# HpWang-whu/YOHO

Measured on AMD Instinct MI355X. Metric: keypoints/sec (5000 kp x60 rot desc+YOHO-O), higher is better.
Workload: dtype fp16x2 split (2^-22-accurate products, fp32 accumulate); 1 GPU

## Files before the change

### yoho_amd/csrc/api.hip

```cpp
#include "common.h"
#include <cstdarg>
#include <cstdio>
#include <cstring>
#include <cstdlib>
#include <cmath>
#include <vector>

namespace yoho {

static thread_local char g_err[512] = "";

void set_error(const char* fmt, ...) {
    va_list ap;
    va_start(ap, fmt);
    vsnprintf(g_err, sizeof(g_err), fmt, ap);
    va_end(ap);
}

void clear_error() { g_err[0] = 0; }

int hip_fail(hipError_t e, const char* what, const char* file, int line) {
    set_error("HIP error %d (%s) at %s:%d: %s", (int)e, hipGetErrorString(e), file, line, what);
    return YOHO_EHIP;
}
// ... 247 lines not shown
                const int* pr = p32.data() + (a < G ? a : G - 1) * G + 4 * q;
                pq[q * 64 + a] = (unsigned)pr[0] | ((unsigned)pr[1] << 8) | ((unsigned)pr[2] << 16) | ((unsigned)pr[3] << 24);
            }
        if ((rc = upload(pq.data(), sizeof(unsigned) * pq.size(), (void**)&c->dPq))) { delete c; return rc; }
    }
    {
        int e = -1;
        for (int g = 0; g < G && e < 0; ++g) {
            float d = 0.f;
            for (int i = 0; i < 9; ++i) d += std::fabs(R[g * 9 + i] - ((i % 4 == 0) ? 1.f : 0.f));
            if (d < 1e-4f) e = g;
        }
        bool ok = e >= 0;
        for (int k = 0; k < NTAP && ok; ++k) {
            const int nk = N[e * NTAP + k];
            int k2 = -1;
            for (int j = 0; j < NTAP; ++j) if (N[nk * NTAP + j] == e) k2 = j;
            if (k2 < 0) ok = false; else c->tap_inv[k] = k2;
        }
        if (!ok) for (int k = 0; k < NTAP; ++k) c->tap_inv[k] = -1;
        if ((rc = upload(c->tap_inv, sizeof(int) * NTAP, (void**)&c->d_tap_inv))) { delete c; return rc; }
    }
    std::vector<int> slab(NCFG * NTAP * G, 0), outg(NCFG * G, -1);
    auto fill = [&](int cfg, const std::vector<int>& glist, int gpw, bool replicate) {
        const int nslots = 4 * gpw;
        for (int sl = 0; sl < nslots; ++sl) {
            int g = -1;
            if (replicate) g = glist[0];
            else if (sl < (int)glist.size()) g = glist[sl];
            outg[cfg * G + sl] = g;
        }
        for (int tap = 0; tap < NTAP; ++tap)
            for (int sl = 0; sl < nslots; ++sl) {
                const int g = outg[cfg * G + sl];
                slab[cfg * NTAP * G + tap * nslots + sl] = (g < 0 ? 0 : (int)N[g * NTAP + tap]) * 1024;
            }
    };
    std::vector<int> all(G); for (int i = 0; i < G; ++i) all[i] = i;
    std::vector<int> one(NTAP); for (int k = 0; k < NTAP; ++k) one[k] = N[k];
    std::vector<bool> in2(G, false);
    for (int k = 0; k < NTAP; ++k) for (int k2 = 0; k2 < NTAP; ++k2) in2[N[one[k] * NTAP + k2]] = true;
    std::vector<int> two; for (int g = 0; g < G; ++g) if (in2[g]) two.push_back(g);
    if (two.size() > 48) { set_error("2-hop cone of group element 0 has %zu > 48 elements", two.size()); delete c; return YOHO_EINVAL; }
    fill(CFG_FULL, all, 15, false);
    fill(CFG_C45, two, 12, false);
    fill(CFG_C13, one, 4, false);
    fill(CFG_C1, std::vector<int>{0}, 1, true);
    if ((rc = upload_slot_tables(slab.data(), outg.data(), c->tabs)) || (rc = gconv_init())) { delete c; return rc; }
    {
        std::vector<int> slab4(3 * 7 * 32, 0), unitg(3 * 32 * 2, -1);
        const std::vector<int>* lists[3] = {&all, &two, &one};
        for (int cfg = 0; cfg < 3; ++cfg) {
            const std::vector<int>& gl = *lists[cfg];
            int* ug = &unitg[cfg * 64];
            for (size_t k = 0; k < gl.size(); ++k) ug[k] = gl[k];
            for (int tp = 0; tp < 7; ++tp)
                for (int u = 0; u < 32; ++u)
                    for (int gs = 0; gs < 2; ++gs)
                        for (int h = 0; h < 2; ++h) {
                            int g = ug[2 * u + gs];
                            if (g < 0) g = ug[2 * u];
                            int tap = 2 * tp + h;
                            if (tap >= NTAP) tap = 2 * tp;
                            slab4[(cfg * 7 + tp) * 32 + u] |= (g < 0 ? 0 : (int)N[g * NTAP + tap]) << (8 * (2 * gs + h));
                        }
        }
        if ((rc = upload_slot_tables16(slab4.data(), unitg.data(), c->tabs)) || (rc = gconv16_init())) { delete c; return rc; }
    }
    c->gconv_mode = 4;
    c->partII_mode = 2;
    {
        auto is = [](const char* name, const char* val) { const char* e = std::getenv(name); return e && std::strcmp(e, val) == 0; };
        auto num = [](const char* name) { const char* e = std::getenv(name); return e ? std::atoi(e) : 0; };
        c->env.partII_tail_staged = is("YOHO_PARTII_TAIL", "staged");
        c->env.transfer_staged = is("YOHO_TRANSFER", "staged");
        c->env.xf_steal = !is("YOHO_XF_STEAL", "0");
        c->env.nn_splits = num("YOHO_NN_SPLITS");
        c->env.fcgf_f32 = is("YOHO_FCGF", "f32");
        c->env.fcgf_full_maps = is("YOHO_FCGF_MAPS", "full");
        c->env.fcgf_norm_staged = is("YOHO_FCGF_NORM", "staged");
        c->env.fcgf_heads_staged = is("YOHO_FCGF_HEADS", "staged");
        if (const char* e = std::getenv("YOHO_WS_LIMIT_MB")) c->env.ws_limit_mb = std::atoll(e);
        if (is("YOHO_PARTII_L1", "3")) c->env.partII_l1_variant = FG_TILE256_W8;
    }
    if (const char* m = std::getenv("YOHO_FCGF_CELLS")) c->fcgf_cell_sort = std::atoi(m);
    if (const char* m = std::getenv("YOHO_FCGF_SORT")) c->fcgf_parity_sort = std::strcmp(m, "0") == 0 ? 0 : 1;
    if (const char* m = std::getenv("YOHO_FCGF_COORDS")) c->fcgf_hash_coords = std::strcmp(m, "hash") == 0 ? 1 : 0;
    if (const char* m = std::getenv("YOHO_NN")) c->nn_prefilter = std::strcmp(m, "brute") == 0 ? 0 : 1;
    if (const char* m = std::getenv("YOHO_PARTII")) c->partII_mode = std::strcmp(m, "f32") == 0 ? 0 : (std::strcmp(m, "fp16x2") == 0 ? 2 : (std::strcmp(m, "cgemm") == 0 ? 3 : (std::strcmp(m, "cgemm8") == 0 ? 4 : 1)));
    if (const char* m = std::getenv("YOHO_PARTI_CHUNK")) {
        int ck = 0, ns = 1;
        if (std::sscanf(m, "%dx%d", &ck, &ns) >= 1 && ck >= 0 && (ns == 1 || ns == 2)) { c->partI_chunk = (ck + 255) / 256 * 256; c->partI_streams = ns; }
    }
    if (const char* m = std::getenv("YOHO_GCONV")) c->gconv_mode = std::strcmp(m, "f32") == 0 ? 0 : (std::strcmp(m, "bf16x3") == 0 ? 1 : (std::strcmp(m, "fp16x2") == 0 ? 3 : (std::strcmp(m, "fgemm") == 0 ? 4 : (std::strcmp(m, "fgemm256") == 0 ? 5 : (std::strcmp(m, "fgemm128") == 0 ? 6 : (std::strcmp(m, "fgemm8") == 0 ? 7 : 2))))));
    c->fb = new FourierBasis();
    if ((rc = build_fourier(N, P, *c->fb))) { delete c->fb; delete c; return rc; }
    {
        std::vector<float> fpad(2 * 64 * 64, 0.f);
        for (int s = 0; s < G; ++s)
            for (int g = 0; g < G; ++g) {
                fpad[s * 64 + g] = (float)c->fb->F[s * G + g];
                fpad[64 * 64 + g * 64 + s] = (float)c->fb->F[s * G + g];
            }
        if ((rc = upload(fpad.data(), fpad.size() * sizeof(float), (void**)&c->dFpad)) || (rc = gft_init()) || (rc = fgemm_init()) || (rc = gft16_init())) { delete c->fb; delete c; return rc; }
        std::vector<unsigned short> f16;
        build_gft16_frags(*c->fb, f16);
        if ((rc = upload(f16.data(), f16.size() * sizeof(unsigned short), &c->dF16))) { delete c->fb; delete c; return rc; }
        hipDeviceProp_t prop;
        if (hipGetDeviceProperties(&prop, device) == hipSuccess && prop.multiProcessorCount > 0) c->nCU = prop.multiProcessorCount;
    }
    HIPCHK(hipMalloc((void**)&c->d_rflag, 4 * sizeof(int)));
    HIPCHK(hipMemset(c->d_rflag, 0, 4 * sizeof(int)));
    HIPCHK(hipMalloc((void**)&c->d_amax, 12 * sizeof(unsigned)));
    HIPCHK(hipMemset(c->d_amax, 0, 12 * sizeof(unsigned)));
    {
        for (int g = 0; g < G; ++g) c->cone_slot_of[g] = -1;
        for (int j = 0; j < NTAP; ++j)
            for (int k = 0; k < NTAP; ++k) c->cone_slot_of[c->hN[c->hN[j] * NTAP + k]] = 0;
        int ns = 0;
        for (int g = 0; g < G; ++g) if (c->cone_slot_of[g] == 0) c->cone_slot_of[g] = ns++;
        c->cone_nslot = ns;
        for (int j = 0; j < NTAP; ++j) {
            c->cone_outg[j] = c->hN[j];
            for (int k = 0; k < NTAP; ++k) c->cone_slot[j * 13 + k] = (unsigned char)c->cone_slot_of[c->hN[c->hN[j] * NTAP + k]];
        }
    }
    HIPCHK(hipMalloc((void**)&c->d_xfctr, 16 * sizeof(int)));
    HIPCHK(hipMemset(c->d_xfctr, 0, 16 * sizeof(int)));
    *out = c;
    return 0;
}

int yoho_ctx_destroy(yoho_ctx* c) {
    if (!c) return 0;
    (void)hipSetDevice(c->device);
    (void)hipDeviceSynchronize();
    for (auto& L : c->p1) free_layer(L);
    for (auto& L : c->p2) free_layer(L);
    if (c->p2_init_bn_s) (void)hipFree(c->p2_init_bn_s);
    if (c->p2_init_bn_t) (void)hipFree(c->p2_init_bn_t);
    if (c->ws.p) (void)hipFree(c->ws.p);
    if (c->dR32) (void)hipFree(c->dR32);
    if (c->dR64) (void)hipFree(c->dR64);
    if (c->dN) (void)hipFree(c->dN);
    if (c->dP) (void)hipFree(c->dP);
    if (c->dPq) (void)hipFree(c->dPq);
    if (c->pair_ws) (void)hipFree(c->pair_ws);
    if (c->pair_host) (void)hipHostFree(c->pair_host);
    if (c->dFpad) (void)hipFree(c->dFpad);
    if (c->dF16) (void)hipFree(c->dF16);
    if (c->fcgf) fcgf_free(c->fcgf);
    if (c->d_tap_inv) (void)hipFree(c->d_tap_inv);
    if (c->d_rflag) (void)hipFree(c->d_rflag);
    if (c->d_xfctr) (void)hipFree(c->d_xfctr);
    if (c->d_amax) (void)hipFree(c->d_amax);
    for (int* t : {c->tabs.slabtab, c->tabs.outg, c->tabs.slab4, c->tabs.unitg}) if (t) (void)hipFree(t);
    delete c->fb;
    for (auto& e : c->ev) (void)hipEventDestroy(e);
    for (auto& e : c->ev_pass) if (e) (void)hipEventDestroy(e);
    for (auto& e : c->phase.pool) (void)hipEventDestroy(e);
    if (c->ev_fork) (void)hipEventDestroy(c->ev_fork);
    if (c->ev_join) (void)hipEventDestroy(c->ev_join);
    if (c->side_stream) (void)hipStreamDestroy(c->side_stream);
    delete c;
    return 0;
}

int yoho_load_partI(yoho_ctx* c, const yoho_partI_weights* w) {
    if (!c || !w) { set_error("yoho_load_partI: null argument"); return YOHO_EINVAL; }
    HIPCHK(hipSetDevice(c->device));
    c->has_partI = false;
    int rc;
    if ((rc = build_layer(c->p1[0], w->conv_in, 32, 256, NTAP, &w->res_in_bn, c->fb))) return rc;
    if ((rc = build_layer(c->p1[1], w->res_in, 256, 512, NTAP, &w->res_out_bn, c->fb))) return rc;
    if ((rc = build_layer(c->p1[2], w->res_out, 512, 256, NTAP, &w->out_bn, c->fb))) return rc;
    if ((rc = build_layer(c->p1[3], w->conv_out, 256, 32, NTAP, nullptr, c->fb))) return rc;
    for (auto& L : c->p1) L.tabs = &c->tabs;
    c->has_partI = true;
    return 0;
}

int yoho_load_partII(yoho_ctx* c, const yoho_partII_weights* w) {
    if (!c || !w) { set_error("yoho_load_partII: null argument"); return YOHO_EINVAL; }
    HIPCHK(hipSetDevice(c->device));
    c->has_partII = false;
    int rc;
    std::vector<float> s, t;
    if (!w->init_bn.gamma || !w->init_bn.beta || !w->init_bn.mean || !w->init_bn.var) { set_error("null batch-norm pointer"); return YOHO_EINVAL; }
    bn_affine(w->init_bn, 128, 128, s, t);
    if (c->p2_init_bn_s) { (void)hipFree(c->p2_init_bn_s); c->p2_init_bn_s = nullptr; }
    if (c->p2_init_bn_t) { (void)hipFree(c->p2_init_bn_t); c->p2_init_bn_t = nullptr; }
    if ((rc = upload(s.data(), 128 * sizeof(float), (void**)&c->p2_init_bn_s))) return rc;
    if ((rc = upload(t.data(), 128 * sizeof(float), (void**)&c->p2_init_bn_t))) return rc;
    if ((rc = build_layer(c->p2[0], w->init, 128, 256, NTAP, &w->res_in_bn, c->fb))) return rc;
    if ((rc = build_layer(c->p2[1], w->res_in, 256, 512, NTAP, &w->res_out_bn))) return rc;
    {
        std::vector<unsigned short> wc, wc8;
        if (pack_cgemm_weights(w->res_in.weight, 256, 512, NTAP, wc, &c->p2[1].wcg_descale, wc8)) { set_error("cone-GEMM weight packing failed"); return YOHO_EINVAL; }
        if ((rc = upload(wc.data(), wc.size() * sizeof(unsigned short), &c->p2[1].wcg))) return rc;
        if ((rc = upload(wc8.data(), wc8.size() * sizeof(unsigned short), &c->p2[1].wcg8))) return rc;
    }
    if ((rc = build_layer(c->p2[2], w->res_out, 512, 256, NTAP, nullptr))) return rc;
    if ((rc = build_layer(c->p2[3], w->fc0, 256, 512, 1, &w->fc0_bn))) return rc;
    if ((rc = build_layer(c->p2[4], w->fc1, 512, 128, 1, &w->fc1_bn))) return rc;
    if ((rc = build_layer(c->p2[5], w->fc2, 128, 4, 1, nullptr))) return rc;
    for (auto& L : c->p2) L.tabs = &c->tabs;
    c->has_partII = true;
    return 0;
}

int yoho_set_gconv_mode(yoho_ctx* c, int mode) {
    if (!c || mode < 0 || mode > 7) { set_error("yoho_set_gconv_mode: mode must be 0 (fp32 MFMA), 1 (bf16x3 MFMA), 2 (group-Fourier fp32 MFMA), 3 (fp16x2 MFMA), 4 (group-Fourier irrep GEMMs, fp16x2 MFMA), 5 or 6 (4 with the other two GEMM blockings), 7 (4 with fp8 correction products)"); return YOHO_EINVAL; }
    c->gconv_mode = mode;
    return 0;
}

int yoho_set_partI_schedule(yoho_ctx* c, int chunk_kp, int streams) {
    if (!c || chunk_kp < 0 || streams < 1 || streams > 2) { set_error("yoho_set_partI_schedule: chunk_kp >= 0 and streams 1 or 2"); return YOHO_EINVAL; }
    c->partI_chunk = (chunk_kp + 255) / 256 * 256;
    c->partI_streams = streams;
    return 0;
}

int yoho_set_partII_mode(yoho_ctx* c, int mode) {
    if (!c || mode < 0 || mode > 4) { set_error("yoho_set_partII_mode: mode must be 0 (fp32 MFMA), 1 (bf16x3), 2 (fp16x2 MFMA, direct cone kernels), 3 (fp16x2, 13-element cone layer as an implicit GEMM) or 4 (3 with fp8 correction products)"); return YOHO_EINVAL; }
    c->partII_mode = mode;
    return 0;
}

int yoho_set_nn_prefilter(yoho_ctx* c, int enable) {
    if (!c) { set_error("yoho_set_nn_prefilter: null ctx"); return YOHO_EINVAL; }
    c->nn_prefilter = enable ? 1 : 0;
    return 0;
}

int yoho_set_fcgf_sort(yoho_ctx* c, int parity_sort, int cell_sort) {
    if (!c) { set_error("yoho_set_fcgf_sort: null ctx"); return YOHO_EINVAL; }
    c->fcgf_parity_sort = parity_sort ? 1 : 0;
    c->fcgf_hash_coords = (cell_sort >= 0 && (cell_sort & 4)) ? 1 : 0;
    cell_sort = cell_sort < 0 ? 0 : (cell_sort & 3);
    c->fcgf_cell_sort = cell_sort > 2 ? 2 : cell_sort;
    return 0;
}

int yoho_set_nn_grid(yoho_ctx* c, double cell) {
    if (!c || !(cell >= 0.0) || !std::isfinite(cell)) { set_error("yoho_set_nn_grid: cell must be a finite number >= 0 (0 = brute force)"); return YOHO_EINVAL; }
    c->nn_cell = cell;
    return 0;
}

int yoho_poison_scratch(yoho_ctx* c, unsigned pattern, void* stream) {
    if (!c) { set_error("yoho_poison_scratch: null ctx"); return YOHO_EINVAL; }
    HIPCHK(hipSetDevice(c->device));
    hipStream_t s = (hipStream_t)stream;
    c->poison = true;
    c->poison_pattern = pattern;
    if (c->ws.p) HIPCHK(hipMemsetD32Async(c->ws.p, (int)pattern, c->ws.bytes / 4, s));
    if (c->pair_ws) HIPCHK(hipMemsetD32Async(c->pair_ws, (int)pattern, c->pair_ws_bytes / 4, s));
    return 0;
}

int yoho_range_status(yoho_ctx* c, int* partI_overflow, int* partII_overflow, void* stream) {
    if (!c) { set_error("yoho_range_status: null ctx"); return YOHO_EINVAL; }
    HIPCHK(hipSetDevice(c->device));
    hipStream_t s = (hipStream_t)stream;
    int h[2] = {0, 0};
    HIPCHK(hipMemcpyAsync(h, c->d_rflag, sizeof(h), hipMemcpyDeviceToHost, s));
    HIPCHK(hipStreamSynchronize(s));
    if (!partI_overflow) h[0] = 0;
    if (!partII_overflow) h[1] = 0;
    if (h[0]) HIPCHK(hipMemsetAsync(c->d_rflag, 0, sizeof(int), s));
    if (h[1]) HIPCHK(hipMemsetAsync(c->d_rflag + 1, 0, sizeof(int), s));
    if (partI_overflow) *partI_overflow = h[0];
    if (partII_overflow) *partII_overflow = h[1];
    if (h[0] || h[1]) {
        set_error("fp16 range exceeded in the fp16x2 arithmetic of %s%s%s since the last check: repeat the pass in mode 1 (bf16x3) or 0 (f32)",
                  h[0] ? "PartI" : "", (h[0] && h[1]) ? " and " : "", h[1] ? "PartII" : "");
        return YOHO_ERANGE;
    }
    return 0;
}

static int ensure_events(yoho_ctx* c, int nchunks) {
    while ((int)c->ev.size() < nchunks * EV_PER_PASS) {
        hipEvent_t e;
        HIPCHK(hipEventCreate(&e));
        c->ev.push_back(e);
    }
    for (auto& e : c->ev_pass) if (!e) HIPCHK(hipEventCreate(&e));
    c->ev_created = true;
    return 0;
}

int yoho_set_profiling(yoho_ctx* c, int enable) {
    if (!c) { set_error("null ctx"); return YOHO_EINVAL; }
    HIPCHK(hipSetDevice(c->device));
    if (enable) { int rc = ensure_events(c, 1); if (rc) return rc; }
    c->profiling = enable != 0;
    c->ev_chunks = 0;
    for (auto& m : c->kernel_ms) m = -1.f;
    return 0;
}

int yoho_phase_profile(yoho_ctx* c, int enable) {
    if (!c) { set_error("null ctx"); return YOHO_EINVAL; }
    PhaseProf& p = c->phase;
    p.on = enable != 0;
    p.used = 0; p.spans.clear(); p.open_cat = -1;
// ... 233 lines not shown
        hipStream_t sk = on_side ? c->side_stream : s;
        char* ws = (char*)c->ws.p + (dbg_own ? slice * (size_t)k : (on_side ? slice : 0));
        if ((rc = partI_passG_chunk(c, ws, slice, k * EV_PER_PASS, xc, n, eqv + (size_t)off * F * G, inv ? inv + (size_t)off * F : nullptr,
                                    inv_np ? inv_np + (size_t)off * F : nullptr, sk, x1c, B0c, on_side ? 1 : 0))) break;
        if (dbg_serial && hipStreamSynchronize(sk) != hipSuccess) { set_error("hipStreamSynchronize failed"); rc = YOHO_EHIP; break; }
    }
    if (nstr == 2) {
        HIPCHK(hipEventRecord(c->ev_join, c->side_stream));
        HIPCHK(hipStreamWaitEvent(s, c->ev_join, 0));
    }
    if (rc) return rc;
    if (prof) (void)hipEventRecord(c->ev_pass[1], s);
    return 0;
}

static int partI_pass(yoho_ctx* c, const float* x, int B, float* eqv, float* inv, float* inv_np, hipStream_t s) {
    if (c->gconv_mode >= 4) return partI_passG(c, x, B, eqv, inv, inv_np, s);
    if (c->gconv_mode == 1 || c->gconv_mode == 3) return partI_pass16(c, x, B, eqv, inv, inv_np, s, c->gconv_mode == 1 ? 3 : 2);
    if (c->gconv_mode == 2) return partI_passF(c, x, B, eqv, inv, inv_np, s);
    const int nT = (B + TILE - 1) / TILE;
    const size_t nX = (size_t)nT * 4, n256 = (size_t)nT * 32, n512 = (size_t)nT * 64;
    int rc;
    float *bX = nullptr, *bH0 = nullptr, *bA = nullptr, *bA1 = nullptr, *bY = nullptr;
    if ((rc = bind_ws(c, s, [&](Arena& ar) {
            bX = ar.take<float>(nX * CHUNK_FLOATS);
            bH0 = ar.take<float>(n256 * CHUNK_FLOATS);
            bA = ar.take<float>(n256 * CHUNK_FLOATS);
            bA1 = ar.take<float>(n512 * CHUNK_FLOATS);
            bY = ar.take<float>(nX * CHUNK_FLOATS);
        }))) return rc;
    const bool prof = c->profiling && c->ev_created;
    auto mark = [&](int i) { if (prof) (void)hipEventRecord(c->ev[i], s); };
    if (prof) { c->ev_chunks = 1; (void)hipEventRecord(c->ev_pass[0], s); }
    mark(0);
    if ((rc = launch_pack_partI(x, B, nT, bX, s))) return rc;
    mark(1);
    if ((rc = launch_gconv(conv_args(c->p1[0], bX, nT, nullptr, bH0, bA, false), 15, EPI_RAW | EPI_ACT, s))) return rc;
    mark(2); mark(3);
    if ((rc = launch_gconv(conv_args(c->p1[1], bA, nT, nullptr, nullptr, bA1, false), 15, EPI_ACT, s))) return rc;
    mark(4); mark(5);
    if ((rc = launch_gconv(conv_args(c->p1[2], bA1, nT, bH0, nullptr, bA, false), 15, EPI_RES | EPI_ACT, s))) return rc;
    mark(6); mark(7);
    if ((rc = launch_gconv(conv_args(c->p1[3], bA, nT, nullptr, bY, nullptr, false), 15, EPI_RAW, s))) return rc;
    mark(8); mark(10);
    if ((rc = launch_finalize_partI(bY, x, B, eqv, inv, inv_np, 0, s))) return rc;
    mark(9);
    if (prof) (void)hipEventRecord(c->ev_pass[1], s);
    return 0;
}

int yoho_partI_forward(yoho_ctx* c, const float* x, int B, float* eqv, float* inv, float* inv_np, void* stream) {
    if (!c || !x || !eqv || B < 1) { set_error("yoho_partI_forward: bad argument (B=%d)", B); return YOHO_EINVAL; }
    if (!c->has_partI) { set_error("yoho_partI_forward: PartI weights not loaded"); return YOHO_ENOWEIGHTS; }
    YOHO_NEED_ALIGNED("yoho_partI_forward", 15, x, eqv, inv, inv_np);
    HIPCHK(hipSetDevice(c->device));
    hipStream_t s = (hipStream_t)stream;
    const int MAXB = 16384;
    for (int b0 = 0; b0 < B; b0 += MAXB) {
        const int nb = B - b0 < MAXB ? B - b0 : MAXB;
        int rc = partI_pass(c, x + (size_t)b0 * F * G, nb, eqv + (size_t)b0 * F * G, inv ? inv + (size_t)b0 * F : nullptr,
                            inv_np ? inv_np + (size_t)b0 * F : nullptr, s);
        if (rc) return rc;
    }
    return 0;
}

int yoho_group_mean_np(yoho_ctx* c, const float* eqv, int B, float* out, void* stream) {
    if (!c || !eqv || !out || B < 0) { set_error("yoho_group_mean_np: bad argument"); return YOHO_EINVAL; }
    if (B == 0) return 0;
    YOHO_NEED_ALIGNED("yoho_group_mean_np", 15, eqv, out);
    HIPCHK(hipSetDevice(c->device));
    return launch_group_mean_np(eqv, B, out, (hipStream_t)stream);
}

static bool partII_fourier_head(const yoho_ctx* c) {
    return c->partII_mode >= 2 && c->p2[0].wpg;
}

static int partII_pass16(yoho_ctx* c, const float* s0, const float* s1, const float* s2, const float* s3, const int64_t* idx,
                         int M, float* quat, hipStream_t s, int npl, const int64_t* const* ridx = nullptr, int istride = 1) {
    const int nT16 = (M + 15) / 16, nT = (M + TILE - 1) / TILE;
    const size_t ch16 = (size_t)npl * 15360;
    const size_t n128 = (size_t)nT * 16, n256 = (size_t)nT * 32, n512 = (size_t)nT * 64, n32 = (size_t)nT * 4;
    const size_t szG = c->partII_mode >= 3 ? (size_t)((nT + 7) / 8) * c->cone_nslot * 8 * 32768 : 0;
    const size_t szX = (size_t)nT16 * 16 * ch16, szA0 = std::max((size_t)nT16 * 32 * ch16, szG);
    const size_t szA1p = npl == 2 ? (size_t)nT16 * 64 * ch16 : 0;
    int rc;
    int* rf = c->d_rflag + 1;
    if (ridx && !partII_fourier_head(c)) { set_error("indexed PartII needs the default (fp16x2, Fourier first layer) mode"); return YOHO_EINVAL; }
    const bool fourier_head = npl == 2 && partII_fourier_head(c);
    const int kppad = (M + 255) / 256 * 256;
    char *bX = nullptr, *bA0 = nullptr, *bA1p = nullptr, *bP = nullptr;
    float *bH0 = nullptr, *bA1 = nullptr, *bF = nullptr, *bF0 = nullptr, *bF1 = nullptr, *bQ = nullptr, *bC = nullptr;
    if ((rc = bind_ws(c, s, [&](Arena& ar) {
            bX = ar.take<char>(szX);
            bA0 = ar.take<char>(szA0);
            bA1p = ar.take<char>(szA1p);
            bH0 = ar.take<float>(n256 * CHUNK_FLOATS);
            bA1 = ar.take<float>(n512 * CHUNK_FLOATS);
            bF = ar.take<float>(n256 * CHUNK_FLOATS);
            bF0 = ar.take<float>(n512 * CHUNK_FLOATS);
            bF1 = ar.take<float>(n128 * CHUNK_FLOATS);
            bQ = ar.take<float>(n32 * CHUNK_FLOATS);
            if (fourier_head) {
                bP = ar.take<char>(fgemm_planes_bytes(kppad, 128));
                bC = ar.take<float>(n256 * CHUNK_FLOATS);
            }
        }))) return rc;
    if (fourier_head) {
        if ((rc = launch_head2(s0, s1, s2, s3, idx, c->dP, c->p2_init_bn_s, c->p2_init_bn_t, M, nT, bP, kppad, c->dF16, s, ridx, istride, rf))) return rc;
        if ((rc = launch_fgemm(c->p2[0], bP, kppad, nT, nullptr, bC, 0, s, rf, c->env.partII_l1_variant))) return rc;
        if (c->partII_mode >= 3 && c->p2[1].wcg && !c->env.partII_tail_staged && mlp_head_supported(c->p2[3], c->p2[4], c->p2[5])) {
            const int nslot = c->cone_nslot;
            unsigned* amax = nullptr;
            if (c->partII_mode == 4) {
                amax = c->d_amax + 8;
                HIPCHK(hipMemsetAsync(amax, 0, sizeof(unsigned), s));
            }
            if ((rc = launch_gft16_invg(bC, bH0, bA0, c->cone_slot_of, nslot, c->dF16, c->p2[0].bn_s, c->p2[0].bn_t, nT, 32, c->nCU, s, rf, amax))) return rc;
            if ((rc = launch_cgemm(c->p2[1], bA0, nslot, c->cone_slot, c->cone_outg, nT, nT16, bA1p, s, rf, amax))) return rc;
            int n0[NTAP];
            for (int k = 0; k < NTAP; ++k) n0[k] = c->hN[k];
            if ((rc = launch_cone1(c->p2[2], bA1p, nT, nT16, nullptr, nullptr, n0, s, bF0))) return rc;
            return launch_mlp_head(c->p2[3], c->p2[4], c->p2[5], nullptr, nT, M, quat, s, bF0, &c->p2[2], bH0);
        }
        if ((rc = launch_gft16_invp(bC, bH0, bA0, nT16, c->dF16, c->p2[0].bn_s, c->p2[0].bn_t, nT, 32, c->nCU, s, rf))) return rc;
    } else {
        if ((rc = launch_pack16_partII(s0, s1, s2, s3, idx, c->dP, c->p2_init_bn_s, c->p2_init_bn_t, M, nT16, bX, s, npl, rf))) return rc;
        if ((rc = launch_gconv16(c->p2[0], bX, nT16, nullptr, nullptr, bA0, EPI_RAW32 | EPI_ACT, s, 1, bH0, nullptr, npl, rf))) return rc;
    }
    if (npl == 2) {
        int n0[NTAP];
        for (int k = 0; k < NTAP; ++k) n0[k] = c->hN[k];
        if ((rc = launch_gconv16(c->p2[1], bA0, nT16, nullptr, nullptr, bA1p, EPI_ACT, s, 2, nullptr, nullptr, npl, rf))) return rc;
        if (!c->env.partII_tail_staged && mlp_head_supported(c->p2[3], c->p2[4], c->p2[5])) {
            if ((rc = launch_cone1(c->p2[2], bA1p, nT, nT16, nullptr, nullptr, n0, s, bF0))) return rc;
            return launch_mlp_head(c->p2[3], c->p2[4], c->p2[5], nullptr, nT, M, quat, s, bF0, &c->p2[2], bH0);
        }
        if ((rc = launch_cone1(c->p2[2], bA1p, nT, nT16, bH0, bF, n0, s))) return rc;
    } else {
        if ((rc = launch_gconv16(c->p2[1], bA0, nT16, nullptr, nullptr, nullptr, EPI_ACT32, s, 2, nullptr, bA1, npl))) return rc;
        if ((rc = launch_gconv(conv_args(c->p2[2], bA1, nT, bH0, bF, nullptr, true), -1, EPI_RES | EPI_RAW, s))) return rc;
    }
    if (!c->env.partII_tail_staged && mlp_head_supported(c->p2[3], c->p2[4], c->p2[5])) return launch_mlp_head(c->p2[3], c->p2[4], c->p2[5], bF, nT, M, quat, s);
    if ((rc = launch_gconv(conv_args(c->p2[3], bF, nT, nullptr, nullptr, bF0, true), -1, EPI_ACT, s))) return rc;
    if ((rc = launch_gconv(conv_args(c->p2[4], bF0, nT, nullptr, nullptr, bF1, true), -1, EPI_ACT, s))) return rc;
    if ((rc = launch_gconv(conv_args(c->p2[5], bF1, nT, nullptr, bQ, nullptr, false), 1, EPI_RAW, s))) return rc;
    return launch_quat_norm(bQ, M, quat, s);
}

static int partII_pass(yoho_ctx* c, const float* s0, const float* s1, const float* s2, const float* s3, const int64_t* idx,
                       int M, float* quat, hipStream_t s) {
    if (c->partII_mode != 0) return partII_pass16(c, s0, s1, s2, s3, idx, M, quat, s, c->partII_mode == 1 ? 3 : 2);
    const int nT = (M + TILE - 1) / TILE;
    const size_t n128 = (size_t)nT * 16, n256 = (size_t)nT * 32, n512 = (size_t)nT * 64, n32 = (size_t)nT * 4;
    int rc;
    float *bX = nullptr, *bH0 = nullptr, *bA0 = nullptr, *bA1 = nullptr, *bF = nullptr, *bF0 = nullptr, *bF1 = nullptr, *bQ = nullptr;
    if ((rc = bind_ws(c, s, [&](Arena& ar) {
            bX = ar.take<float>(n128 * CHUNK_FLOATS);
            bH0 = ar.take<float>(n256 * CHUNK_FLOATS);
            bA0 = ar.take<float>(n256 * CHUNK_FLOATS);
            bA1 = ar.take<float>(n512 * CHUNK_FLOATS);
            bF = ar.take<float>(n256 * CHUNK_FLOATS);
            bF0 = ar.take<float>(n512 * CHUNK_FLOATS);
            bF1 = ar.take<float>(n128 * CHUNK_FLOATS);
            bQ = ar.take<float>(n32 * CHUNK_FLOATS);
        }))) return rc;
    if ((rc = launch_pack_partII(s0, s1, s2, s3, idx, c->dP, c->p2_init_bn_s, c->p2_init_bn_t, M, nT, bX, s))) return rc;
    if ((rc = launch_gconv(conv_args(c->p2[0], bX, nT, nullptr, bH0, bA0, false), 12, EPI_RAW | EPI_ACT, s))) return rc;
    if ((rc = launch_gconv(conv_args(c->p2[1], bA0, nT, nullptr, nullptr, bA1, false), 4, EPI_ACT, s))) return rc;
    if ((rc = launch_gconv(conv_args(c->p2[2], bA1, nT, bH0, bF, nullptr, true), -1, EPI_RES | EPI_RAW, s))) return rc;
    if (!c->env.partII_tail_staged && mlp_head_supported(c->p2[3], c->p2[4], c->p2[5])) return launch_mlp_head(c->p2[3], c->p2[4], c->p2[5], bF, nT, M, quat, s);
    if ((rc = launch_gconv(conv_args(c->p2[3], bF, nT, nullptr, nullptr, bF0, true), -1, EPI_ACT, s))) return rc;
    if ((rc = launch_gconv(conv_args(c->p2[4], bF0, nT, nullptr, nullptr, bF1, true), -1, EPI_ACT, s))) return rc;
    if ((rc = launch_gconv(conv_args(c->p2[5], bF1, nT, nullptr, bQ, nullptr, false), 1, EPI_RAW, s))) return rc;
    return launch_quat_norm(bQ, M, quat, s);
}

int yoho_partII_forward(yoho_ctx* c, const float* before_eqv0, const float* before_eqv1, const float* after_eqv0,
                        const float* after_eqv1, const int64_t* pre_idx, int M, float* quat, void* stream) {
    if (!c || M < 0) { set_error("yoho_partII_forward: bad argument"); return YOHO_EINVAL; }
    if (!c->has_partII) { set_error("yoho_partII_forward: PartII weights not loaded"); return YOHO_ENOWEIGHTS; }
    if (M == 0) return 0;
    if (!before_eqv0 || !before_eqv1 || !after_eqv0 || !after_eqv1 || !pre_idx || !quat) {
        set_error("yoho_partII_forward: bad argument"); return YOHO_EINVAL;
    }
    YOHO_NEED_ALIGNED("yoho_partII_forward", 15, before_eqv0, before_eqv1, after_eqv0, after_eqv1, quat);
    YOHO_NEED_ALIGNED("yoho_partII_forward", 7, pre_idx);
    HIPCHK(hipSetDevice(c->device));
    hipStream_t s = (hipStream_t)stream;
    const int MAXM = 8192;
    for (int m0 = 0; m0 < M; m0 += MAXM) {
        const int nm = M - m0 < MAXM ? M - m0 : MAXM;
        const size_t o = (size_t)m0 * F * G;
        int rc = partII_pass(c, before_eqv0 + o, before_eqv1 + o, after_eqv0 + o, after_eqv1 + o, pre_idx + m0, nm,
// ... 210 lines not shown
```

### yoho_amd/csrc/common.h

```cpp
#pragma once
#include <hip/hip_runtime.h>
#include <stdint.h>
#include <stddef.h>
#include <initializer_list>
#include "yoho_hip.h"
#include "arena.h"

namespace yoho {

constexpr int G = 60;
constexpr int NTAP = 13;
constexpr int F = 32;
constexpr int TILE = 32;
constexpr int SLAB_FLOATS = 2 * TILE * 4;
constexpr int CHUNK_FLOATS = G * SLAB_FLOATS;

void set_error(const char* fmt, ...);
void clear_error();
inline bool yoho_misaligned(std::initializer_list<const void*> ps, unsigned mask) {
    for (const void* p : ps) if ((reinterpret_cast<uintptr_t>(p) & mask) != 0) return true;
    return false;
}
#define YOHO_NEED_ALIGNED(fn, mask, ...)                                                                                  \
    do {                                                                                                                  \
// ... 151 lines not shown
int launch_gconv16(const Layer& L, const char* X, int nTiles, const float* res, float* out_raw, char* out_act, int flags, hipStream_t s,
                   int cfg = 0, float* out_raw32 = nullptr, float* out_act32 = nullptr, int npl = 3, int* rflag = nullptr);
int launch_pack16_partII(const float* s0, const float* s1, const float* s2, const float* s3, const int64_t* pre_idx, const int* P,
                         const float* bn_s, const float* bn_t, int M, int nTiles16, char* out, hipStream_t s, int npl = 3, int* rflag = nullptr);
int launch_pack16_partI(const float* x, int B, int nTiles, char* out, hipStream_t s, int npl = 3, int* rflag = nullptr);
int launch_group_mean_np(const float* eqv, int B, float* out, hipStream_t s);
int launch_pack_partII(const float* s0, const float* s1, const float* s2, const float* s3, const int64_t* pre_idx,
                       const int* P, const float* bn_s, const float* bn_t, int M, int nTiles, float* out, hipStream_t s);
int launch_quat_norm(const float* y, int M, float* quat, hipStream_t s);

struct MfArgs {
    const float* a; const float* b;
    int Na, Nb;
    float* na2; float* nb2;
    _Float16* a16; _Float16* b16;
    unsigned* rowmin; unsigned* colmin;
    unsigned long long* keysA; unsigned long long* keysB;
    unsigned* maxn2;
    int* bad;
    int tilesPer;
    unsigned long long* cand;
    unsigned* ncand; unsigned cap;
};
void mutual_prefilter_layout(Arena& ar, int Na, int Nb, MfArgs& p);
int launch_mutual_prefilter(MfArgs& p, const float* a, const float* b, int nCU, hipStream_t s, int nn_splits = 0);
int launch_nn32seg(const float* src, int Ns, const float* tgt, int Nt, int D, int dist_type, int nCU, unsigned long long* keys, bool init_keys,
                   const int* run_if, int64_t* idx, float* dist, hipStream_t s);
struct GridWs {
    unsigned long long* keys; int* head; unsigned cap;
    int* next; int* ulist; int* ucount;
};
void grid_nn_layout(Arena& ar, int Ns, int Nt, GridWs& w);
void grid_transfer_layout(Arena& ar, int K, int nb, int mmax, GridWs& w);
int launch_grid_transfer_batch(const double* pts, const int64_t* kidx, int K, const double* R_host, int nb, const float* const* ds,
                               const float* const* feat, const int* m, int g0, float* out, double cell, const GridWs& w, int nCU, hipStream_t s);
struct Workspace;
}
struct yoho_ctx;
namespace yoho {
int ensure_ws(yoho_ctx* ctx, size_t bytes, hipStream_t s);
struct GnMat3;
int launch_grid_nn(int mode, const void* src, int Ns, const GnMat3* R, const float* tgt, int Nt, double cell, const GridWs& w, int64_t* idx, float* dist,
                   double* part_d, int* part_i, int nCU, hipStream_t s);

struct Workspace {
    void* p = nullptr;
    size_t bytes = 0;
};

inline const char* experiment_env(const char* name) {
#ifdef YOHO_EXPERIMENTS
    return std::getenv(name);
#else
    (void)name;
    return nullptr;
#endif
}

struct PhaseProf {
    static constexpr int NCAT = 16;
    bool on = false;
    std::vector<hipEvent_t> pool;
    size_t used = 0;
    struct Span { int cat; hipEvent_t a, b; };
    std::vector<Span> spans;
    int open_cat = -1;
    hipEvent_t open_ev = nullptr;
    double flops[NCAT] = {0};
    double launches[NCAT] = {0};
};

}

struct yoho_env_switches {
    bool partII_tail_staged = false;
    bool transfer_staged = false;
    bool xf_steal = true;
    int nn_splits = 0;
    bool fcgf_f32 = false;
    bool fcgf_full_maps = false;
    bool fcgf_norm_staged = false;
    bool fcgf_heads_staged = false;
    yoho::FGemmBlocking partII_l1_variant = yoho::FG_TILE128;
    long long ws_limit_mb = 0;
};

struct yoho_ctx {
    int device = 0;
    yoho_env_switches env;
    float* dR32 = nullptr;
    double* dR64 = nullptr;
    int* dN = nullptr;
    int* dP = nullptr;
    unsigned* dPq = nullptr;
    uint8_t hN[60 * 13];
    uint8_t hP[60 * 60];
    float hR[60 * 9];
    bool has_partI = false, has_partII = false;
    yoho::Layer p1[4];
    yoho::Layer p2[6];
    float *p2_init_bn_s = nullptr, *p2_init_bn_t = nullptr;
    int partII_mode = 2;
    int cone_nslot = 0;
    int cone_slot_of[60];
    unsigned char cone_slot[13 * 13];
    unsigned char cone_outg[13];
    int gconv_mode = 4;
    yoho::FourierBasis* fb = nullptr;
    float* dFpad = nullptr;
    void* dF16 = nullptr;
    yoho::FcgfNet* fcgf = nullptr;
    int tap_inv[13] = {0};
    int* d_tap_inv = nullptr;
    int nCU = 256;
    yoho::SlotTables tabs;
    int* d_rflag = nullptr;
    unsigned* d_amax = nullptr;
    int* d_xfctr = nullptr;
    int fcgf_cell_sort = 1;
    int fcgf_hash_coords = 0;
    int fcgf_parity_sort = 1;
    int nn_prefilter = 1;
    double nn_cell = 0.0;
    yoho::Workspace ws;
    void* pair_ws = nullptr; size_t pair_ws_bytes = 0;
    bool poison = false; unsigned poison_pattern = 0;
    void* pair_host = nullptr; size_t pair_host_bytes = 0;
    int partI_chunk = 0;
    int partI_streams = 1;
    hipStream_t side_stream = nullptr;
    hipEvent_t ev_fork = nullptr, ev_join = nullptr;
    bool profiling = false;
    std::vector<hipEvent_t> ev;
    int ev_chunks = 0;
    hipEvent_t ev_pass[2] = {nullptr, nullptr};
    bool ev_created = false;
    float kernel_ms[8];
    yoho::PhaseProf phase;
};
namespace yoho {
inline void phase_mark(yoho_ctx* c, int cat, hipStream_t s) {
    PhaseProf& p = c->phase;
    if (!p.on) return;
    if (p.open_cat < 0 && cat < 0) return;
    if (p.used == p.pool.size()) {
        hipEvent_t e;
        if (hipEventCreate(&e) != hipSuccess) return;
        p.pool.push_back(e);
    }
    hipEvent_t e = p.pool[p.used++];
    (void)hipEventRecord(e, s);
    if (p.open_cat >= 0) p.spans.push_back({p.open_cat, p.open_ev, e});
    p.open_cat = cat < PhaseProf::NCAT ? cat : -1;
    p.open_ev = e;
}
inline void phase_work(yoho_ctx* c, int cat, double flops) {
    if (c->phase.on && cat >= 0 && cat < PhaseProf::NCAT) { c->phase.flops[cat] += flops; c->phase.launches[cat] += 1.0; }
}
}
namespace yoho { constexpr int EV_PER_PASS = 11; }

namespace yoho {
template <typename Lay>
int bind_ws(yoho_ctx* ctx, hipStream_t s, Lay&& lay) {
    Arena measure;
    lay(measure);
// ... 13 lines not shown
```

### yoho_amd/csrc/gemmf2.hip

```cpp
#include <hip/hip_runtime.h>
#include <cstdlib>
#include <cstring>
#include "common.h"
#include "gemmf.h"

namespace yoho {

constexpr int F2_BUF = 24576;
constexpr int F2_LDS = 3 * F2_BUF;
constexpr int F3_BUF = 32768;
constexpr int F3_LDS = 3 * F3_BUF;

struct Frags2 {
    uintx4 ah[4], al[4], bh[2], bl[2];
};

template <int LO, int R>
__device__ __forceinline__ void read_frag2(const char* pa, const char* pb, Frags2& f) {
    if constexpr (R < 4) f.al[R] = *reinterpret_cast<const uintx4*>(pa + 8192 + R * 512);
    else if constexpr (R < 6) f.bh[R - 4] = *reinterpret_cast<const uintx4*>(pb + (R - 4) * 512);
    else if constexpr (R < 10) f.ah[R - 6] = *reinterpret_cast<const uintx4*>(pa + (R - 6) * 512);
    else f.bl[R - 10] = *reinterpret_cast<const uintx4*>(pb + LO + (R - 10) * 512);
}
template <int LO>
// ... 544 lines not shown
    const unsigned* amax;
    unsigned char slot[13 * 13];
    unsigned char outg[16];
};

__device__ __forceinline__ void cg_split_pair(float x0, float x1, unsigned& hi, unsigned& lo) {
    typedef float f2 __attribute__((ext_vector_type(2)));
    f2 x;
    x.x = x0; x.y = x1;
    const halfx2 h = __builtin_convertvector(x, halfx2);
    const f2 r = x - __builtin_convertvector(h, f2);
    const halfx2 l = __builtin_convertvector(r, halfx2);
    __builtin_memcpy(&hi, &h, 4);
    __builtin_memcpy(&lo, &l, 4);
}

template <bool FP8>
__global__ __launch_bounds__(512, 2) void cgemm_kernel(CGemmArgs a) {
    extern __shared__ __attribute__((aligned(16))) char smem[];
    __shared__ int tapoff[16];
    const int tid = threadIdx.x, lane = tid & 63;
    const Wave3 wv(__builtin_amdgcn_readfirstlane(tid >> 6), lane);
    const int xcd = blockIdx.x & 7, slot_ = blockIdx.x >> 3;
    const int ct = xcd + 8 * (slot_ / a.MT), mtile = slot_ % a.MT;
    if (ct >= a.nj * a.NTm) return;
    const int j = ct / a.NTm, mt = ct - j * a.NTm;
    const int SPT = 2 * a.KSt;
    const int KT = a.ntap * SPT;
    if (tid < 16) tapoff[tid] = tid < a.ntap ? (int)a.slot[j * 13 + tid] : 0;
    const char* Ag = a.A + (size_t)mtile * (KT / 2) * FG_STAGE;
    const char* Bt = a.B + (size_t)mt * a.nslot * a.KSt * FG_STAGE;
    __syncthreads();
    auto bsrc = [&](int s) -> const char* {
        const int tap = s / SPT, within = s - tap * SPT;
        const int sl = __builtin_amdgcn_readfirstlane(tapoff[tap]);
        return Bt + (size_t)sl * a.KSt * FG_STAGE + step_off(within);
    };

    floatx16 acc[4][2];
    zero_acc(acc);
    C8Scales sc;
    if constexpr (FP8) sc = C8Scales(a.amax);
    dma_step(wv.dm, Ag, uniform_ptr(bsrc(0)), smem);
    dma_step(wv.dm, Ag + step_off(1), uniform_ptr(bsrc(1)), smem + F3_BUF);
    asm volatile("s_waitcnt vmcnt(0)" ::: "memory");
    __builtin_amdgcn_s_barrier();

    ring_plain<FP8>(acc, smem, wv, Ag, bsrc, KT, true, sc);

    const int half = lane >> 5, c32 = lane & 31;
    const int g = a.outg[j];
    unsigned top = 0u;
#pragma unroll
    for (int bi = 0; bi < 2; ++bi) {
        const int m = mt * 256 + wv.nh * 128 + wv.wn * 64 + bi * 32 + c32;
        if ((m >> 5) >= a.nT32 || (m >> 4) >= a.nTiles16) continue;
#pragma unroll
        for (int ai = 0; ai < 4; ++ai) {
#pragma unroll
            for (int q4 = 0; q4 < 4; ++q4) {
                const int o = mtile * 256 + wv.wm * 128 + ai * 32 + q4 * 8 + half * 4;
                const floatx4 b4 = *reinterpret_cast<const floatx4*>(a.bias + o);
                const floatx4 s4 = *reinterpret_cast<const floatx4*>(a.bn_s + o);
                const floatx4 t4 = *reinterpret_cast<const floatx4*>(a.bn_t + o);
                float y[4];
#pragma unroll
                for (int e = 0; e < 4; ++e) {
                    const float v = acc[ai][bi][4 * q4 + e] * a.descale + b4[e];
                    y[e] = fmaxf(v * s4[e] + t4[e], 0.f) * H2_ASCALE;
                    top = max(top, __float_as_uint(y[e]) & 0x7FFFFFFFu);
                }
                unsigned h0, l0, h1, l1;
                cg_split_pair(y[0], y[1], h0, l0);
                cg_split_pair(y[2], y[3], h1, l1);
                char* dst = a.out + (((size_t)(m >> 4) * a.c8out + (o >> 3)) * 2) * 15360 + g * 256 + (m & 15) * 16 + half * 8;
                *reinterpret_cast<uint2*>(dst) = uint2{h0, h1};
                *reinterpret_cast<uint2*>(dst + 15360) = uint2{l0, l1};
            }
        }
    }
    note_range_bits(a.rflag, top, FP16_MAX);
}

int cgemm_init() {
    HIPCHK(hipFuncSetAttribute(reinterpret_cast<const void*>(&cgemm_kernel<true>), hipFuncAttributeMaxDynamicSharedMemorySize, F3_LDS));
    HIPCHK(hipFuncSetAttribute(reinterpret_cast<const void*>(&cgemm_kernel<false>), hipFuncAttributeMaxDynamicSharedMemorySize, F3_LDS));
    return 0;
}

int launch_cgemm(const Layer& L, const char* Bstages, int nslot, const unsigned char* slot, const unsigned char* outg, int nT32, int nTiles16,
                 char* out, hipStream_t s, int* rflag, const unsigned* amax) {
    const bool fp8 = amax != nullptr;
    if (!(fp8 ? L.wcg8 : L.wcg) || L.cin % 32 || L.cout % 256) { set_error("cgemm: needs the cone-GEMM weight pack, cin %% 32 == 0, cout %% 256 == 0"); return YOHO_EINVAL; }
    if (nT32 == 0) return 0;
    CGemmArgs a;
    a.A = reinterpret_cast<const char*>(fp8 ? L.wcg8 : L.wcg); a.B = Bstages; a.bias = L.bias; a.bn_s = L.bn_s; a.bn_t = L.bn_t; a.out = out;
    a.NTm = (nT32 + 7) / 8; a.MT = L.cout / 256; a.KSt = L.cin / 32; a.ntap = 13; a.nj = 13; a.nslot = nslot; a.c8out = L.cout / 8;
    a.nT32 = nT32; a.nTiles16 = nTiles16; a.descale = L.wcg_descale; a.rflag = rflag; a.amax = amax;
    std::memcpy(a.slot, slot, 169);
    std::memset(a.outg, 0, 16);
    std::memcpy(a.outg, outg, 13);
    const int CT = a.nj * a.NTm;
    const int grid = 8 * ((CT + 7) / 8) * a.MT;
    if (fp8) hipLaunchKernelGGL(cgemm_kernel<true>, dim3(grid), dim3(512), F3_LDS, s, a);
    else hipLaunchKernelGGL(cgemm_kernel<false>, dim3(grid), dim3(512), F3_LDS, s, a);
    HIPCHK(hipGetLastError());
    return 0;
}

struct Frags3s {
    uintx4 ah[5], al[5], bh, bl;
};

template <int R>
__device__ __forceinline__ void read_frag3s(const char* pa, const char* pb, Frags3s& f) {
    if constexpr (R < 5) f.al[R] = *reinterpret_cast<const uintx4*>(pa + 8192 + R * 512);
    else if constexpr (R == 5) f.bh = *reinterpret_cast<const uintx4*>(pb);
    else if constexpr (R < 11) f.ah[R - 6] = *reinterpret_cast<const uintx4*>(pa + (R - 6) * 512);
    else f.bl = *reinterpret_cast<const uintx4*>(pb + 8192);
}

template <bool DMA, int D>
__device__ __forceinline__ void step3s(const Frags3s& f, floatx16 (&acc)[5][1], const char* ra, const char* rb, Frags3s& nf,
                                       const char* srcA, const char* srcB, char* dmabuf, const Dma3& dm) {
    sfor<0, 5>([&](auto gc) {
        constexpr int g = decltype(gc)::value;
        if constexpr (g < D) acc[g][0] = mfma_h(f.al[g], f.bh, acc[g][0]);
        if constexpr (g < D) read_frag3s<g>(ra, rb, nf);
        if constexpr (g == 4) read_frag3s<5>(ra, rb, nf);
        __builtin_amdgcn_sched_barrier(0);
    });
    sfor<0, 5>([&](auto gc) {
        constexpr int g = decltype(gc)::value;
        if constexpr (g < D) acc[g][0] = mfma_h(f.ah[g], f.bl, acc[g][0]);
        if constexpr (g < D) read_frag3s<6 + g>(ra, rb, nf);
        if constexpr (g == 4) read_frag3s<11>(ra, rb, nf);
        __builtin_amdgcn_sched_barrier(0);
    });
    sfor<0, 5>([&](auto gc) {
        constexpr int g = decltype(gc)::value;
        if constexpr (g < D) acc[g][0] = mfma_h(f.ah[g], f.bh, acc[g][0]);
        if constexpr (DMA && g < 4) dm.template piece<g>(srcA, srcB, dmabuf);
        __builtin_amdgcn_sched_barrier(0);
    });
}

template <int D>
__device__ __forceinline__ void fgemm3s_kloop(floatx16 (&acc)[5][1], char* smem, const char* Ag, const char* Bg, int KT, const Dma3& dm, int lane_a, int lane_b) {
    Frags3s P;
    sfor<0, 12>([&](auto rc) {
        constexpr int R = decltype(rc)::value;
        if constexpr (R == 5 || R == 11 || (R < 5 && R < D) || (R > 5 && R < 11 && R - 6 < D)) read_frag3s<R>(smem + lane_a, smem + lane_b, P);
    });
    ring_pipelined<F3_BUF, 4>(smem, Ag, Bg, KT, lane_a, lane_b, P,
        [&](auto dmac, const Frags3s& f, Frags3s& nf, const char* ra, const char* rb, const char* srcA, const char* srcB, char* buf) {
            step3s<decltype(dmac)::value, D>(f, acc, ra, rb, nf, srcA, srcB, buf, dm);
        });
}

__global__ __launch_bounds__(512, 2) void fgemm3s_kernel(FGemmArgs a, int flags) {
    extern __shared__ __attribute__((aligned(16))) char smem[];
    const int tid = threadIdx.x, lane = tid & 63;
    const int w8 = __builtin_amdgcn_readfirstlane(tid >> 6);
    int t = 0, local = 0, r = 0;
    if (!fg3_map(a, blockIdx.x & 7, blockIdx.x >> 3, t, local, r)) return;
    const int d = a.dim[t];
    const int KS = d * a.cin / 32, KT = 2 * KS;
    const int ntile = r + 8 * local;
    const char* Ag = a.A + a.a_off[t];
    const char* Bg = a.B + a.b_off[t] + (size_t)ntile * KS * FG_STAGE;
    const Dma3 dm(w8, lane);
    const int lane_a = (lane >> 5) * 4096 + (lane & 31) * 16;
    const int lane_b = 16384 + (lane >> 5) * 4096 + (w8 * 32 + (lane & 31)) * 16;

    floatx16 acc[5][1];
    zero_acc(acc);
    ring_prologue<F3_BUF>(KT, [&](int st, int buf) { dma_step(dm, uniform_ptr(Ag + step_off(st)), uniform_ptr(Bg + step_off(st)), smem + buf); });
    asm volatile("s_waitcnt vmcnt(0)" ::: "memory");
    __builtin_amdgcn_s_barrier();

    switch (d) {
        case 1: fgemm3s_kloop<1>(acc, smem, Ag, Bg, KT, dm, lane_a, lane_b); break;
        case 3: fgemm3s_kloop<3>(acc, smem, Ag, Bg, KT, dm, lane_a, lane_b); break;
        case 4: fgemm3s_kloop<4>(acc, smem, Ag, Bg, KT, dm, lane_a, lane_b); break;
        default: fgemm3s_kloop<5>(acc, smem, Ag, Bg, KT, dm, lane_a, lane_b); break;
    }
    const int colbase = ntile * 256 + w8 * 32;
// ... 51 lines not shown
```

Before: 1.908 million keypoints/s.

## Default PartII fp16x2 to cone implicit GEMM and add K32-step cone GEMM kernel

Makes partII mode 2 (the default) route the 13-element cone layer through the implicit-GEMM path unless YOHO_PARTII_CONE=direct, instead of the direct cone kernels. It also adds a cone GEMM kernel that processes 32-deep K steps with double-buffered DMA and register-prefetched fragments, and uses it for non-fp8 launches whenever the stage count is even. The aim is to cut the direct cone kernel cost and per-step pipeline overhead. The cost is a larger workspace for the gathered cone slots and a new kernel path whose correctness depends on helpers defined elsewhere.

New measurement: 1.931 million keypoints/s (median of 6 runs). +1.2%, better.

```diff
diff --git a/yoho_amd/csrc/api.hip b/yoho_amd/csrc/api.hip
--- a/yoho_amd/csrc/api.hip
+++ b/yoho_amd/csrc/api.hip
@@ -353,6 +353,7 @@
         c->env.fcgf_heads_staged = is("YOHO_FCGF_HEADS", "staged");
         if (const char* e = std::getenv("YOHO_WS_LIMIT_MB")) c->env.ws_limit_mb = std::atoll(e);
         if (is("YOHO_PARTII_L1", "3")) c->env.partII_l1_variant = FG_TILE256_W8;
+        c->env.partII_cone_direct = is("YOHO_PARTII_CONE", "direct");
     }
     if (const char* m = std::getenv("YOHO_FCGF_CELLS")) c->fcgf_cell_sort = std::atoi(m);
     if (const char* m = std::getenv("YOHO_FCGF_SORT")) c->fcgf_parity_sort = std::strcmp(m, "0") == 0 ? 0 : 1;
@@ -494,7 +495,7 @@
 }
 
 int yoho_set_partII_mode(yoho_ctx* c, int mode) {
-    if (!c || mode < 0 || mode > 4) { set_error("yoho_set_partII_mode: mode must be 0 (fp32 MFMA), 1 (bf16x3), 2 (fp16x2 MFMA, direct cone kernels), 3 (fp16x2, 13-element cone layer as an implicit GEMM) or 4 (3 with fp8 correction products)"); return YOHO_EINVAL; }
+    if (!c || mode < 0 || mode > 4) { set_error("yoho_set_partII_mode: mode must be 0 (fp32 MFMA), 1 (bf16x3), 2 (fp16x2 MFMA, 13-element cone layer as an implicit GEMM unless YOHO_PARTII_CONE=direct), 3 (2 with the cone GEMM whatever that switch says) or 4 (3 with fp8 correction products)"); return YOHO_EINVAL; }
     c->partII_mode = mode;
     return 0;
 }
@@ -894,7 +895,8 @@
     const int nT16 = (M + 15) / 16, nT = (M + TILE - 1) / TILE;
     const size_t ch16 = (size_t)npl * 15360;
     const size_t n128 = (size_t)nT * 16, n256 = (size_t)nT * 32, n512 = (size_t)nT * 64, n32 = (size_t)nT * 4;
-    const size_t szG = c->partII_mode >= 3 ? (size_t)((nT + 7) / 8) * c->cone_nslot * 8 * 32768 : 0;
+    const bool cone_gemm = c->partII_mode >= 3 || (c->partII_mode == 2 && !c->env.partII_cone_direct);
+    const size_t szG = cone_gemm ? (size_t)((nT + 7) / 8) * c->cone_nslot * 8 * 32768 : 0;
     const size_t szX = (size_t)nT16 * 16 * ch16, szA0 = std::max((size_t)nT16 * 32 * ch16, szG);
     const size_t szA1p = npl == 2 ? (size_t)nT16 * 64 * ch16 : 0;
     int rc;
@@ -922,7 +924,7 @@
     if (fourier_head) {
         if ((rc = launch_head2(s0, s1, s2, s3, idx, c->dP, c->p2_init_bn_s, c->p2_init_bn_t, M, nT, bP, kppad, c->dF16, s, ridx, istride, rf))) return rc;
         if ((rc = launch_fgemm(c->p2[0], bP, kppad, nT, nullptr, bC, 0, s, rf, c->env.partII_l1_variant))) return rc;
-        if (c->partII_mode >= 3 && c->p2[1].wcg && !c->env.partII_tail_staged && mlp_head_supported(c->p2[3], c->p2[4], c->p2[5])) {
+        if (cone_gemm && c->p2[1].wcg && !c->env.partII_tail_staged && mlp_head_supported(c->p2[3], c->p2[4], c->p2[5])) {
             const int nslot = c->cone_nslot;
             unsigned* amax = nullptr;
             if (c->partII_mode == 4) {
diff --git a/yoho_amd/csrc/common.h b/yoho_amd/csrc/common.h
--- a/yoho_amd/csrc/common.h
+++ b/yoho_amd/csrc/common.h
@@ -257,6 +257,7 @@
     bool fcgf_norm_staged = false;
     bool fcgf_heads_staged = false;
     yoho::FGemmBlocking partII_l1_variant = yoho::FG_TILE128;
+    bool partII_cone_direct = false;
     long long ws_limit_mb = 0;
 };
 
diff --git a/yoho_amd/csrc/gemmf2.hip b/yoho_amd/csrc/gemmf2.hip
--- a/yoho_amd/csrc/gemmf2.hip
+++ b/yoho_amd/csrc/gemmf2.hip
@@ -650,9 +650,102 @@
     note_range_bits(a.rflag, top, FP16_MAX);
 }
 
+__global__ __launch_bounds__(512, 2) void cgemmk_kernel(CGemmArgs a) {
+    extern __shared__ __attribute__((aligned(16))) char smem[];
+    __shared__ int tapoff[16];
+    const int tid = threadIdx.x, lane = tid & 63;
+    const int w8 = __builtin_amdgcn_readfirstlane(tid >> 6);
+    const int xcd = blockIdx.x & 7, slot_ = blockIdx.x >> 3;
+    const int ct = xcd + 8 * (slot_ / a.MT), mtile = slot_ % a.MT;
+    if (ct >= a.nj * a.NTm) return;
+    const int j = ct / a.NTm, mt = ct - j * a.NTm;
+    const int KS = a.ntap * a.KSt;
+    if (tid < 16) tapoff[tid] = tid < a.ntap ? (int)a.slot[j * 13 + tid] : 0;
+    const char* Ag = a.A + (size_t)mtile * KS * FG_STAGE;
+    const char* Bt = a.B + (size_t)mt * a.nslot * a.KSt * FG_STAGE;
+    __syncthreads();
+    auto bsrc = [&](int st) -> const char* {
+        const int tap = st / a.KSt, cb = st - tap * a.KSt;
+        const int sl = __builtin_amdgcn_readfirstlane(tapoff[tap]);
+        return uniform_ptr(Bt + ((size_t)sl * a.KSt + cb) * FG_STAGE);
+    };
+    const int wm = (w8 & 3) >> 1, wn = w8 & 1, nh = w8 >> 2;
+    const Dma3k dm(w8, lane);
+    const int lane_a = (lane >> 4) * 4096 + (wm * 128 + (lane & 15)) * 16;
+    const int lane_b = FG_STAGE + (lane >> 4) * 4096 + (nh * 128 + wn * 64 + (lane & 15)) * 16;
+
+    floatx4 acc[8][4];
+    zero_acc(acc);
+    auto dma = [&](int st, int buf) {
+        const char* sa = uniform_ptr(Ag + (size_t)st * FG_STAGE);
+        const char* sb = bsrc(st);
+        sfor<0, Dma3k::NP>([&](auto uc) { dm.template piece<decltype(uc)::value>(sa, sb, smem + buf); });
+    };
+    dma(0, 0);
+    dma(1, F3K_BUF);
+    asm volatile("s_waitcnt vmcnt(0)" ::: "memory");
+    __builtin_amdgcn_s_barrier();
+
+    FragsA32 fa[2];
+    FragsB32 P, Q;
+    sfor<0, 10>([&](auto rc) { read_open32<decltype(rc)::value>(smem + lane_a, smem + lane_b, fa[0], P); });
+    int s = 0, cur = 0;
+    auto run = [&](auto dmac, const FragsB32& b, FragsB32& nb) {
+        const int nxt = cur ^ F3K_BUF;
+        if constexpr (decltype(dmac)::value)
+            step32<true>(dm, acc, fa, b, nb, smem + cur + lane_a, smem + nxt + lane_a, smem + nxt + lane_b, uniform_ptr(Ag + (size_t)(s + 2) * FG_STAGE),
+                         bsrc(s + 2), smem + cur);
+        else
+            step32<false>(dm, acc, fa, b, nb, smem + cur + lane_a, smem + nxt + lane_a, smem + nxt + lane_b, nullptr, nullptr, nullptr);
+        cur = nxt; ++s;
+    };
+    constexpr std::true_type dmay;
+    constexpr std::false_type dman;
+    while (s + 2 < KS) {
+        run(dmay, P, Q);
+        run(dmay, Q, P);
+    }
+    run(dman, P, Q);
+    run(dman, Q, P);
+
+    int etid = threadIdx.x;
+    asm volatile("" : "+v"(etid));
+    const int g4 = (etid >> 4) & 3, c16 = etid & 15;
+    const int g = a.outg[j];
+    const int col0 = mt * 256 + nh * 128 + wn * 64;
+    unsigned top = 0u;
+#pragma unroll
+    for (int ai = 0; ai < 8; ++ai) {
+        const int o = mtile * 256 + wm * 128 + ai * 16 + g4 * 4;
+        const floatx4 b4 = *reinterpret_cast<const floatx4*>(a.bias + o);
+        const floatx4 s4 = *reinterpret_cast<const floatx4*>(a.bn_s + o);
+        const floatx4 t4 = *reinterpret_cast<const floatx4*>(a.bn_t + o);
+#pragma unroll
+        for (int bi = 0; bi < 4; ++bi) {
+            const int m0 = col0 + bi * 16;
+            if ((m0 >> 5) >= a.nT32 || (m0 >> 4) >= a.nTiles16) continue;
+            float y[4];
+#pragma unroll
+            for (int e = 0; e < 4; ++e) {
+                const float v = acc[ai][bi][e] * a.descale + b4[e];
+                y[e] = fmaxf(v * s4[e] + t4[e], 0.f) * H2_ASCALE;
+                top = max(top, __float_as_uint(y[e]) & 0x7FFFFFFFu);
+            }
+            unsigned h0, l0, h1, l1;
+            cg_split_pair(y[0], y[1], h0, l0);
+            cg_split_pair(y[2], y[3], h1, l1);
+            char* dst = a.out + (((size_t)(m0 >> 4) * a.c8out + (o >> 3)) * 2) * 15360 + g * 256 + c16 * 16 + (g4 & 1) * 8;
+            *reinterpret_cast<uint2*>(dst) = uint2{h0, h1};
+            *reinterpret_cast<uint2*>(dst + 15360) = uint2{l0, l1};
+        }
+    }
+    note_range_bits(a.rflag, top, FP16_MAX);
+}
+
 int cgemm_init() {
     HIPCHK(hipFuncSetAttribute(reinterpret_cast<const void*>(&cgemm_kernel<true>), hipFuncAttributeMaxDynamicSharedMemorySize, F3_LDS));
     HIPCHK(hipFuncSetAttribute(reinterpret_cast<const void*>(&cgemm_kernel<false>), hipFuncAttributeMaxDynamicSharedMemorySize, F3_LDS));
+    HIPCHK(hipFuncSetAttribute(reinterpret_cast<const void*>(&cgemmk_kernel), hipFuncAttributeMaxDynamicSharedMemorySize, F3K_LDS));
     return 0;
 }
 
@@ -670,7 +763,10 @@
     std::memcpy(a.outg, outg, 13);
     const int CT = a.nj * a.NTm;
     const int grid = 8 * ((CT + 7) / 8) * a.MT;
+    const char* dbg = experiment_env("YOHO_FGEMM_DEBUG");
+    const bool k32 = !fp8 && (a.ntap * a.KSt) % 2 == 0 && !(dbg && std::strstr(dbg, "k16"));
     if (fp8) hipLaunchKernelGGL(cgemm_kernel<true>, dim3(grid), dim3(512), F3_LDS, s, a);
+    else if (k32) hipLaunchKernelGGL(cgemmk_kernel, dim3(grid), dim3(512), F3K_LDS, s, a);
     else hipLaunchKernelGGL(cgemm_kernel<false>, dim3(grid), dim3(512), F3_LDS, s, a);
     HIPCHK(hipGetLastError());
     return 0;
```
